# nv-tlabs/ASE

Measured on AMD Instinct MI355X. Metric: ASE PPO-update samples/sec (4096 envs x horizon 32), higher is better.
Workload: dtype f16; 1 GPU; BASELINE configs[1]: ASE agent, 4096 envs x horizon 32, obs 253 / act 31 / amp obs 1400 / latent 64, [1024,1024,512] MLPs + disc + shared-trunk encoder, minibatch 16384 (amp 4096) x 6 mini-epochs = 48 optimisation steps per update; random-init weights; precision_choice=auto without an oracle leg: the first candidate, replay=program, parallelism=single GPU

## Files before the change

ase_amd/backend.py:

```python
import ctypes as C

import torch

from . import lib as L


_HOSTFN = C.CFUNCTYPE(None, C.c_void_p)


def _ptr(t):
    return None if t is None else C.c_void_p(t.data_ptr())


def _ld(t):
    return 0 if t is None else int(t.stride(0))


def _code(dtype):
    if dtype == torch.bfloat16:
        return L.BF16
    if dtype == torch.float32:
        return L.F32
    if dtype == torch.float16:
        return L.F16
    raise L.AseHipError(f"unsupported storage dtype {dtype}")


class HipBackend:
    name = "hip"
    nt_fused_epilogue = True

    def __init__(self, device=None, x3=False):
        self.x3 = x3 if x3 == 'f16' else bool(x3)
        self._recording, self._host_keep, self._host_error = None, {}, None
        self.tn_workspace = True
        if not torch.cuda.is_available():
            raise L.AseHipError("HipBackend needs a ROCm GPU (torch.cuda.is_available() is False); "
                                "the update path has no CPU fallback")
        self.device = torch.device(device if device is not None else f"cuda:{torch.cuda.current_device()}")
        self.lib = L.get()
        self._head_scratch = torch.zeros(L.PPO_SCRATCH, dtype=torch.float64, device=self.device)
        self._head_scratch_ls = None

    def _stream(self):
        return C.c_void_p(torch.cuda.current_stream(self.device).cuda_stream)

    def zero_(self, t):
        assert t.is_contiguous()
        L.check(self.lib.ase_hip_memset(_ptr(t), 0, t.numel() * t.element_size(), self._stream()), "memset")

    def copy_(self, dst, src):
        assert dst.is_contiguous() and src.is_contiguous() and dst.dtype == src.dtype and dst.numel() == src.numel()
        L.check(self.lib.ase_hip_memcpy(_ptr(dst), _ptr(src), dst.numel() * dst.element_size(), self._stream()), "memcpy")
# ... 104 lines not shown
            row = [A.data_ptr(), _ld(A), B.data_ptr(), _ld(B), G.data_ptr(), 0 if gb is None else gb.data_ptr(), int(br),
                   M, N, K, nr, kr, ss, sd, struct.unpack('<i', struct.pack('<f', float(alpha)))[0], 0]
            for j, v in enumerate(row):
                tab[16 * i + j] = int(v)
        max_work = 8192
        work = (C.c_int32 * (4 * max_work))()
        red = (C.c_int32 * (4 * max_work))()
        n_work, n_red = C.c_int(0), C.c_int(0)
        L.check(self.lib.ase_hip_gemm_tn_grouped_plan(tab, n, int(target_wg), work, max_work, C.byref(n_work), red, max_work,
                                                      C.byref(n_red)), "gemm_tn_grouped_plan")
        nw, nr = n_work.value, n_red.value
        dev_tab = torch.tensor(list(tab), dtype=torch.int64, device=self.device)
        dev_work = torch.tensor(list(work[:4 * nw]), dtype=torch.int32, device=self.device)
        dev_red = torch.tensor(list(red[:4 * nr]), dtype=torch.int32, device=self.device)
        ws = torch.empty(nw * L.TN_SLAB, dtype=torch.float32, device=self.device) if self.tn_workspace else None
        return {'problems': dev_tab, 'work': dev_work, 'n_work': nw, 'red': dev_red, 'n_red': nr, 'ws': ws, 'keep': problems,
                'dtype': _code(problems[0][0].dtype), 'alpha_dev': alpha_dev}

    def gemm_tn_grouped(self, plan):
        L.check(self.lib.ase_hip_gemm_tn_grouped(_ptr(plan['problems']), _ptr(plan['work']), plan['n_work'], _ptr(plan['red']),
                                                 plan['n_red'], _ptr(plan['ws']), _ptr(plan.get('alpha_dev')), plan['dtype'],
                                                 self._stream()),
                "gemm_tn_grouped")

    def refresh_shadow(self, W, Ws, Wts, split_src, split_dst, x3_exp=None):
        n, k = W.shape
        ref = Ws if Ws is not None else Wts
        code = _code(ref.dtype)
        if x3_exp is not None:
            assert ref.dtype == torch.float32
            code = L.F32H3 | (int(x3_exp) << 16)
        L.check(self.lib.ase_hip_refresh_shadow(_ptr(W), n, k, _ptr(Ws), _ld(Ws), _ptr(Wts), _ld(Wts), split_src,
                                                split_dst, code, self._stream()), "refresh_shadow")

    def refresh_shadow_multi(self, desc, items, dtype):
        L.check(self.lib.ase_hip_refresh_shadow_multi(_ptr(desc), desc.shape[0], _code(dtype), self._stream()),
                "refresh_shadow_multi")

    def apply_multi(self, desc, items, dtype, opt_state, acc):
        L.check(self.lib.ase_hip_apply_multi(_ptr(desc), desc.shape[0], _ptr(opt_state), _ptr(acc), _code(dtype),
                                             self._stream()), "apply_multi")

    def apply_multi_split(self, desc, items, dtype, opt_state, acc, desc2, items2):
        assert desc2.shape == (desc.shape[0], 8) and desc2.is_contiguous()
        L.check(self.lib.ase_hip_apply_multi_v2(_ptr(desc), desc.shape[0], _ptr(desc2), _ptr(opt_state), _ptr(acc), _code(dtype),
                                                self._stream()), "apply_multi_v2")
# ... 362 lines not shown
```

ase_amd/engine.py:

```python
import contextlib
import math

import torch

from . import lib as L


def P(x, m=64):
    return (int(x) + m - 1) // m * m


_ACT = {'relu': L.ACT_RELU, 'tanh': L.ACT_TANH, 'None': L.ACT_NONE, 'none': L.ACT_NONE, None: L.ACT_NONE,
        'swish': L.ACT_SILU, 'silu': L.ACT_SILU, 'elu': L.ACT_ELU, 'gelu': L.ACT_GELU, 'sigmoid': L.ACT_SIGMOID,
        'selu': L.ACT_SELU, 'softplus': L.ACT_SOFTPLUS}
_AUX = {L.ACT_RELU: L.AUX_RELU_MASK, L.ACT_TANH: L.AUX_TANH_GRAD, L.ACT_NONE: L.AUX_NONE}
_AUX.update({a: L.AUX_PREACT | (a << 8) for a in range(L.ACT_SILU, L.ACT_SOFTPLUS + 1)})


class Dense:

    def __init__(self, parts, k_in, act, split=None):
        self.parts = parts
        self.K = k_in
        self.act = _ACT[act] if not isinstance(act, int) else act
# ... 54 lines not shown
        self.bounds_coef = float(cfg.get('bounds_loss_coef') or 0.0)
        self.adaptive_lr = cfg.get('lr_schedule', 'constant') == 'adaptive'
        self.kl_threshold = float(cfg.get('kl_threshold', 0.008))
        self.obs, self.act = net.obs_size, net.actions_num
        self.z = net.latent_dim if kind == 'ase' else 0
        self.amp = net.amp_obs_size if kind in ('amp', 'ase') else 0
        self.masked = kind in ('amp', 'ase')
        self.has_disc = kind in ('amp', 'ase')
        self.has_enc = kind == 'ase'
        self.div_on = kind == 'ase' and cfg.get('amp_diversity_bonus', 0) != 0
        self.enc_sep = bool(getattr(net, 'enc_separate', False))
        self.enc_gp = kind == 'ase' and cfg.get('enc_grad_penalty', 0) != 0 and cfg.get('enc_coef', 0) != 0
        self.mu_tanh = kind == 'ppo' and getattr(net, 'mu_tanh', False)
        self.sigma_mode = getattr(net, 'sigma_mode', 'frozen')
        self.ls_mode = {'frozen': L.LS_FROZEN, 'vector': L.LS_VECTOR, 'head': L.LS_ROWS}[self.sigma_mode]
        self.gp32 = bool(cfg.get('gp_f32', False)) and self.has_disc and dtype in (torch.float16, torch.bfloat16) and \
            cfg.get('disc_coef', 0) * cfg.get('disc_grad_penalty', 0) != 0
        self._scratch = {}
        self.multi_stream = bool(cfg.get('multi_stream', True)) and getattr(backend, 'name', '') == 'hip'
        self._side_streams = None
        o = dict(tn_grouped=True, tn_wg_side=64, tn_early=False, disc_early=True, short_prologue=True, style_early=False,
                 relu_bits=True, fused_apply=True, apply_wide=True, side_streams=2, gp_scale_split=True, xstep=True,
                 gp_stream='auto', style_side=0, style_wg=0, side_priority=None, prefetch=True, disc_after_style=False, gp_split='f16',
                 stream_offset=0, gp_value_late=False, gp_fuse='auto')
        unknown = set(cfg.get('engine_opts', {}) or {}) - set(o)
        assert not unknown, f"unknown engine_opts {sorted(unknown)}"
        o.update(cfg.get('engine_opts', {}) or {})
        self.engine_opts = o
        self._tn_defer = bool(getattr(backend, 'grouped_tn_ok', None)) and bool(o['tn_grouped'])
        self._tn_queue, self._tn_plans = [], {}
        self._tn_wg_side = int(o['tn_wg_side'])
        self._tn_early = bool(o['tn_early'])
        self._disc_early = bool(o['disc_early'])
        self._early_fork = None
        self._short_prologue = bool(o['short_prologue']) and cfg.get('graph_capture') != 'hipgraph'
        self._prep = self._lat_ready = self._fill_done = None
        self._style_early = bool(o['style_early'])
        self._n_side = max(1, min(int(o['side_streams']), 2))
        self._apply_groups = None
        self._use_bits = bool(o['relu_bits'])
        self._fused_apply = hasattr(backend, 'apply_multi') and bool(o['fused_apply'])
        self._xstep = bool(o['xstep']) and cfg.get('graph_capture') != 'hipgraph'
        gp_side = (self.dyn_scale or self.M < 8192) if o['gp_stream'] == 'auto' else bool(o['gp_stream'])
        self._gp_side = gp_side and cfg.get('graph_capture') != 'hipgraph'
        self._gp_fuse = bool(self.gp32 and getattr(backend, 'nt_fused_epilogue', False) and cfg.get('gp_f32') == 'x3'
                             and getattr(backend, 'x3', None) is not None and o['gp_split'] == 'f16'
                             and (o['gp_fuse'] == 'auto' or bool(o['gp_fuse'])))
# ... 7 lines not shown
        self._par, self._par_set, self._last_par, self._fenced = 0, False, None, False
        self._stats_exchanged = False
        self._style_wg = int(o['style_wg'])
        sp = o['side_priority']
        if sp is None:
            sp = [0, -1, 0] if (self.gp32 or self.dyn_scale) else [-1, 0, 0]
        self._side_prio = [int(x) for x in sp] if isinstance(sp, (list, tuple)) else [int(sp)] * 3
        self._gp_stream_obj = None
        self._xs = False
        self._disc_fwd_out = self._gp_value_done = self._pre_done = None
        self._apply_wide = bool(o['apply_wide'])
        self._apply_desc = self._apply_items = None
        self.force_dist = bool(cfg.get('force_dist', False))
        self.dp_grad_dtype = cfg.get('dp_grad_dtype', 'f32')
        assert self.dp_grad_dtype in ('f32', 'bf16'), self.dp_grad_dtype
        self._xbuf = {}
        self._disc_acc_mark = None
        self._merged_stats = False
        self._acc_in_bucket = False
        self._refresh_desc = None
        self._mb_desc = None
        self._mb_desc_key = None
        self._build_layers()
        self._bind_params()
        self._alloc(infer_rows)
        self.refresh_shadows()

    def _build_layers(self):
        net, z = self.net, self.z
        act = net.activation
        split = (self.obs, P(self.obs), P(self.obs) + P(z)) if z else None
        self.style = []
        if self.kind == 'ase':
            k = z
            for i, u in enumerate(net.style_units):
                self.style.append(Dense([(f'actor_mlp._style_mlp.{2 * i}', u, 0)], k, act))
                k = u
            self.style.append(Dense([('actor_mlp._style_dense', z, 0)], k, 'tanh'))
            names_a = [f'actor_mlp._dense_layers.{i}' for i in range(len(net.units))]
            names_c = [f'critic_mlp._mlp.{2 * i}' for i in range(len(net.units))]
        else:
            names_a = [f'actor_mlp.{2 * i}' for i in range(len(net.units))]
            names_c = [f'critic_mlp.{2 * i}' for i in range(len(net.units))]
        self.actor, self.critic = [], []
        k = self.obs + z
        for i, u in enumerate(net.units):
# ... 334 lines not shown
    def _mask_of(self, h):
        e = self._bits.get(h.untyped_storage().data_ptr()) if h is not None else None
        if e is None:
            return None
        base, bits = e
        off = (h.data_ptr() - base.data_ptr()) // base.element_size()
        r0, c0 = divmod(off, base.stride(0))
        if c0 != 0 or h.shape[1] != base.shape[1]:
            return None
        return bits[r0:r0 + h.shape[0]]

    def _twin(self, h, d):
        if d.act >= L.ACT_SILU:
            t = self._mask_of(h)
            assert t is not None
            return t
        return h

    def _fwd_chain(self, chain, X, H, rows):
        for d, h in zip(chain, H):
            self._fwd(d, X, h, rows)
            X = h
        return X

    def _dgrad(self, d, dY, dX, rows, aux, aux_act, wts=None, n_out=None, alpha=1.0):
        wts = d.Wts if wts is None else wts
        n_out = d.k_pad if n_out is None else n_out
        aux, mode = self._aux(aux, _AUX[aux_act])
        self._nt(dY, wts, dX, rows, n_out, d.n_pad, aux=aux, aux_mode=mode, alpha=alpha)

    def _wgrad(self, d, dY, X, rows, alpha=1.0, bias=True):
        heads = len(d.parts) > 1 or d in (self.mu_head, self.value_head, self.disc_head, self.enc_head)
        for (name, nr, off), gW, gb in zip(d.parts, d.gW, d.gb):
            self._tn(dY[:, off:], X, gW, rows, P(nr), d.k_pad, nr, d.K, d.split_src, d.split_dst, alpha=alpha,
                     gbias=gb if (bias and not heads) else None)

    def _tn(self, A, B, G, M, N, K, n_real, k_real, split_src, split_dst, alpha=1.0, gbias=None, bias_rows=0):
        br = bias_rows if bias_rows > 0 else M
        alpha = alpha / self.gs
        if self._tn_defer and self.be.grouped_tn_ok(A.dtype, M, n_real, K, br):
            self._tn_queue.append((A, B, G, gbias, br, M, N, K, n_real, k_real, split_src, split_dst, alpha))
        else:
            self.be.gemm_tn(A, B, G, M, N, K, n_real, k_real, split_src, split_dst, alpha=alpha, gbias=gbias,
                            bias_rows=bias_rows, alpha_dev=self._dI)

    def _flush_tn(self, target_wg=0):
# ... 162 lines not shown
                elif self.masked:
                    be.reduce_sum(self.mb['rand_action_mask'], M, False, self.acc, L.ACC_MASK_SUM)
                    if self._dist_shard():
                        self._ar(self.acc[L.ACC_MASK_SUM:L.ACC_MASK_SUM + 1])
            self._fill_done = None
            self._prep = prep
            self._stats_exchanged = True
            return
        be.begin_step(self.opt_state if advance else None, self.acc,
                      zero2=None if pf else (self.obs_sums if self._xs else self.stats_flat),
                      rng_bump=self.div_rng if (self.div_on and not pf) else None)
        self._prep = None
        if self._short_prologue and self._amp_stats_in_branch():
            m0 = self._mark()
            with self._Branch(self, self._side(1), m0):
                be.zero_(self.grads[:self.n_train])
                self._fill_done = self._mark()
            self._early_fork = self._fill_done if self.has_disc else None
            with self._Branch(self, self._side(0), m0) as prep:
                self.gather_minibatch(ds, idx, remap, part=2)
                if self.div_on:
                    self._draw_new_latents(new_z)
                if self.style and self._style_early:
                    sd = self.actor[0].split_dst
                    h = self._fwd_chain(self.style[:-1], self.Zs, self.Hs, self.Ra)
                    self._fwd(self.style[-1], h, self.Xa[:, sd:], self.Ra)
                self._lat_ready = self._mark()
                self.gather_minibatch(ds, idx, remap, part=1)
                if self.masked:
                    be.reduce_sum(self.mb['rand_action_mask'], M, False, self.acc, L.ACC_MASK_SUM)
            self._prep = prep
            if c.get('normalize_input', True):
                be.rms_moments(ds['obs'], self.obs, idx, remap, M, self.obs_state, self.obs_sums)
            return
        be.zero_(self.grads[:self.n_train])
        self._early_fork = self._mark() if (self.has_disc and self._amp_stats_in_branch() and self._disc_early) else None
        self.gather_minibatch(ds, idx, remap)
        if self.masked:
            be.reduce_sum(self.mb['rand_action_mask'], M, False, self.acc, L.ACC_MASK_SUM)
        if c.get('normalize_input', True):
            be.rms_moments(ds['obs'], self.obs, idx, remap, M, self.obs_state, self.obs_sums)
        if self.has_disc and not self._amp_stats_in_branch():
            self._amp_moments(amp_streams)

    def _amp_stats_in_branch(self):
        return self.multi_stream and not (self._dist_shard() and self.cfg.get('graph_capture') == 'hipgraph')

    def _dist_shard(self):
        return self._dist_on() and self.shard
# ... 166 lines not shown
            hd = he = None
        elif self._disc_fwd_out is not None:
            hd, he = self._disc_fwd_out
        elif disc_early:
            with self._Branch(self, self._side(1), fork0):
                hd, he = self._disc_forward(amp_streams)
        if self._pre_done is None:
            if norm_in:
                be.rms_finalize(self.obs_state, self.obs, self.obs_sums, self.Mg if self.shard else self.M, 1, self.obs_mean,
                                self.obs_std)
            else:
                self._identity_stats(self.obs_mean, self.obs_std)
            outs = [self.Xa[:M], self.Xc]
            if self.div_on:
                outs.append(self.Xa[M:])
            be.rms_normalize(ds['obs'], self.obs, idx, remap, M, self.obs_mean[0], self.obs_std[0], outs)
        fork1 = self._mark()
        if self._prep is not None:
            be.wait(self._lat_ready)
        elif self.div_on:
            self._draw_new_latents(new_z)

        if self.style and not (self._prep is not None and self._style_early and self._pre_done is None):
            sd = self.actor[0].split_dst
            h = self._fwd_chain(self.style[:-1], self.Zs, self.Hs, Ra)
            self._fwd(self.style[-1], h, self.Xa[:, sd:], Ra)
        style_launched = self._mark() if self._disc_fwd_out == 'split' else None
        ha = self._fwd_chain(self.actor, self.Xa, self.Ha, Ra)
        self._fwd(self.mu_head, ha, self.MU, Ra)

        with self._Branch(self, self._side(0), fork1) as br_critic:
            hc = self._fwd_chain(self.critic, self.Xc, self.Hc, M)
            self._fwd(self.value_head, hc, self.V, M)

        br_disc = None
        if self.has_disc:
            tnq, self._tn_queue = self._tn_queue, []
            with self._Branch(self, self._side(1), fork0) as br_disc:
                if self._disc_fwd_out == 'split':
                    be.wait(style_launched)
                    hd, he = self._disc_matrices()
                elif not disc_early:
                    hd, he = self._disc_forward(amp_streams)
                be.disc_head(self.HD, self.dHD, self.disc_head.gb[0], self.acc, AMB, amb_den, c['disc_coef'],
                             grad_scale=self.gs, dyn=self._dS)
                if self.has_enc:
                    src, sidx, srm = amp_streams[0]
                    zsrc = ds['ase_latents'].view(ds['ase_latents'].shape[0], -1)
                    if not self._enc_z_ready:
# ... 44 lines not shown
        self._dgrad(self.mu_head, self.dMU, self.dZa[-1], Ra, self.Ha[-1], last.act)
        self._bwd_chain(self.actor, self.Xa, self.Ha, self.dZa, Ra)
        tn_actor, self._tn_queue = self._tn_queue, []
        actor_done = self._mark()
        with self._Branch(self, self._side(0), fork2) as br_cb:
            self._wgrad(self.value_head, self.dV, hc, M)
            last = self.critic[-1]
            self._dgrad(self.value_head, self.dV, self.dZc[-1], M, self.Hc[-1], last.act)
            self._bwd_chain(self.critic, self.Xc, self.Hc, self.dZc, M)
            if self._tn_early:
                if actor_done is not None:
                    be.wait(actor_done)
                self._tn_queue = tn_actor + self._tn_queue
                self._flush_tn(0)
            else:
                tn_actor = tn_actor + self._tn_queue
                self._tn_queue = []
        def style_backward():
            a0, sdn = self.actor[0], self.style[-1]
            sd = a0.split_dst
            self._dgrad(a0, self.dZa[0], self.dStyle, Ra, self.Xa[:, sd:], sdn.act, wts=a0.Wts[sd:], n_out=P(self.z))
            hs_last = self.Hs[-1] if self.Hs else self.Zs
            self._wgrad(sdn, self.dStyle, hs_last, Ra)
            if self.Hs:
                p = self.style[-2]
                self._dgrad(sdn, self.dStyle, self.dZs[-1], Ra, self.Hs[-1], p.act)
                self._bwd_chain(self.style[:-1], self.Zs, self.Hs, self.dZs, Ra)

        if self.style and self._style_side == 2 and self.multi_stream and self._tn_defer and not self._tn_early:
            self._join_branch(br_cb)
            wide, self._tn_queue = tn_actor, []
            with self._Branch(self, self._side(0), actor_done) as br_style:
                style_backward()
            narrow, self._tn_queue = self._tn_queue, wide
            self._flush_tn(0)
            self._join_branch(br_style)
            self._tn_queue = narrow
        elif self.style and self._style_side and self.multi_stream and self._tn_defer and not self._tn_early:
            self._join_branch(br_cb)
            wide, self._tn_queue = tn_actor, []
            with self._Branch(self, self._side(0), actor_done) as br_style:
                if self._style_wg <= 0:
                    defer, self._tn_defer = self._tn_defer, False
                    style_backward()
                    self._tn_defer = defer
                else:
                    style_backward()
# ... 502 lines not shown
    def _eval_stats(self, state, D, key):
        mean, std = self._scr(key + '_m', 1, D, torch.float32), self._scr(key + '_s', 1, D, torch.float32)
        self.be.rms_finalize(state, D, None, 0, 0, mean, std)
        return mean[0], std[0]

    def _policy_nets(self, obs, z, normalize, want_mu, want_value):
        be, n = self.be, obs.shape[0]
        f32 = torch.float32
        a0 = self.actor[0]
        Xa, Xc = self._scr('Xa', n, a0.k_pad), self._scr('Xc', n, a0.k_pad)
        if normalize and self.cfg.get('normalize_input', True):
            mean, std = self._eval_stats(self.obs_state, self.obs, 'obs')
        else:
            mean, std = self._scr('one_m', 1, self.obs, f32)[0].zero_(), self._scr('one_s', 1, self.obs, f32)[0].fill_(1.0)
        be.rms_normalize(obs, self.obs, None, (0, 0), n, mean, std, [Xa, Xc])
        MU = V = None
        if self.z:
            sd = a0.split_dst
            be.gather_rows(z, self.z, None, (0, 0), n, Xc[:, sd:])
        if want_mu:
            if self.style:
                Zs = self._scr('Zs', n, P(self.z))
                be.gather_rows(z, self.z, None, (0, 0), n, Zs)
                h = Zs
                for i, d in enumerate(self.style[:-1]):
                    y = self._scr(f'Hs{i}', n, d.n_pad)
                    self._fwd(d, h, y, n)
                    h = y
                self._fwd(self.style[-1], h, Xa[:, a0.split_dst:], n)
            h = Xa
            for i, d in enumerate(self.actor):
                y = self._scr(f'Ha{i}', n, d.n_pad)
                self._fwd(d, h, y, n)
                h = y
            MU = self._scr('MU', n, self.mu_head.n_pad, f32)
            self._fwd(self.mu_head, h, MU, n)
        if want_value:
            h = Xc
            for i, d in enumerate(self.critic):
                y = self._scr(f'Hc{i}', n, d.n_pad)
                self._fwd(d, h, y, n)
                h = y
            V = self._scr('V', n, self.value_head.n_pad, f32)
            self._fwd(self.value_head, h, V, n)
        return MU, V

    def _value_out(self, V, n, unnorm_value, key='value_out'):
        v = self._scr(key, n, 1, torch.float32)
        self.be.gather_rows(V, 1, None, (0, 0), n, v)
        if unnorm_value and self.norm_value:
            self.be.rms_unnormalize(self.val_state, v, v)
        return v
# ... 140 lines not shown
```

ase_amd/lib.py:

```python
import ctypes as C
import os

_HERE = os.path.dirname(os.path.abspath(__file__))
LIB_PATH = os.path.join(_HERE, "csrc", "libase_hip.so")

ABI_VERSION = 9
PPO_SCRATCH = 1024 * 72 + 8
PPO_SCRATCH_LS = 1024 * 136 + 8
LS_FROZEN, LS_VECTOR, LS_ROWS = 0, 1, 2
TN_SLAB = 65536 + 256
F32, BF16, F32X3, F16, F32H3 = 0, 1, 2, 3, 4
ACT_NONE, ACT_RELU, ACT_TANH, ACT_SILU, ACT_ELU, ACT_GELU, ACT_SIGMOID, ACT_SELU, ACT_SOFTPLUS = range(9)
AUX_NONE, AUX_RELU_MASK, AUX_TANH_GRAD, AUX_RELU_BITS, AUX_PREACT = 0, 1, 2, 3, 4
TASK_HEADING, TASK_LOCATION, TASK_REACH, TASK_STRIKE = range(4)
TASK_OBS_COLS = (5, 2, 3, 15)
RESET_FRAME, RESET_TABLE, RESET_MOTION = range(3)
RESET_HAS_TABLE, RESET_HAS_MOTION = 1, 2

(ACC_MASK_SUM, ACC_A_LOSS, ACC_B_LOSS, ACC_ENTROPY, ACC_CLIPPED, ACC_C_LOSS, ACC_KL, ACC_DIV, ACC_BCE_AGENT,
 ACC_BCE_DEMO, ACC_AGENT_ACC, ACC_DEMO_ACC, ACC_GP, ACC_ENC, ACC_ENC_GP, ACC_LOGIT_W2, ACC_DISC_W2, ACC_ENC_W2,
 ACC_GRAD_SQ) = range(19)
ACC_COUNT = 24
(RES_A_LOSS, RES_C_LOSS, RES_B_LOSS, RES_ENTROPY, RES_CLIP_FRAC, RES_KL, RES_DISC_LOSS, RES_DISC_GP,
 RES_DISC_LOGIT_LOSS, RES_DISC_AGENT_ACC, RES_DISC_DEMO_ACC, RES_ENC_LOSS, RES_DIV_LOSS, RES_LOSS,
 RES_MASK_SUM, RES_ENC_GP, RES_LR) = range(17)
RES_COUNT = 20

_p, _i, _i64, _f, _d = C.c_void_p, C.c_int, C.c_int64, C.c_float, C.c_double

SIGNATURES = {
    "ase_hip_gemm_nt": [_p, _i64, _p, _i64, _p, _i64, _p, _p, _i64, _i, _i, _p, _i, _p, _i64, _i, _i, _i, _i, _i, _i, _f, _p, _i, _p],
    "ase_hip_gemm_nt_ex": [_p, _i64, _p, _i64, _p, _i64, _p, _p, _i64, _i, _i, _p, _i, _p, _i64, _i, _i, _i, _i, _i, _i, _f, _p, _i,
                           _p, _i, _f, _p, _i64, _i, _p, _d, _p, _p],
    "ase_hip_gemm_tn": [_p, _i64, _p, _i64, _p, _p, _i, _i, _i, _i, _i, _i, _i, _i, _f, _p, _i, _p],
    "ase_hip_refresh_shadow": [_p, _i, _i, _p, _i64, _p, _i64, _i, _i, _i, _p],
    "ase_hip_refresh_shadow_multi": [_p, _i, _i, _p],
    "ase_hip_gather_multi": [_p, _i, _p, _i, _i, _i, _p],
    "ase_hip_rms_moments": [_p, _i64, _i, _p, _i, _i, _i, _p, _p, _p],
    "ase_hip_rms_finalize": [_p, _i, _p, _p, _i, _p, _p, _p],
    "ase_hip_rms_normalize": [_p, _i64, _i, _p, _i, _i, _i, _p, _p, _p, _i64, _p, _i64, _p, _i64, _i, _p],
    "ase_hip_rms_unnormalize": [_p, _p, _p, _i64, _p],
    "ase_hip_gather_rows": [_p, _i64, _i, _p, _i, _i, _i, _p, _i64, _i, _p],
    "ase_hip_reduce_sum": [_p, _i64, _i, _p, _i, _p],
    "ase_hip_ppo_head": [_p, _i64, _p, _i64] + [_p] * 11 + [_p, _i64, _p, _i64, _p, _p, _p, _p, _p] + [_i] * 8 + [_f] * 6 + [_p]
                        + [_i, _i64, _p, _i64, _p, _f] + [_i, _p],
    "ase_hip_disc_head": [_p, _i64, _p, _i64, _p, _p, _i, _i, _f, _f, _p, _i, _p],
    "ase_hip_enc_head": [_p, _i64, _p, _i64, _p, _i64, _p, _p, _p, _i, _i, _i, _f, _f, _p, _i, _p],
    "ase_hip_gp_seed": [_p, _i64, _p, _p, _i64, _i, _i, _f, _i, _i, _p],
    "ase_hip_gp_second": [_p, _i64, _p, _i64, _p, _i64, _p, _i64, _i, _i, _i, _i, _p],
    "ase_hip_colsum": [_p, _i64, _i, _i, _f, _p, _p],
    "ase_hip_sqnorm": [_p, _i64, _i, _i, _p, _i, _d, _p, _i, _p],
    "ase_hip_finalize_scalars": [_p, _p, _i, _i, _i, _i, _i, _i] + [_f] * 11 + [_p, _f, _p],
    "ase_hip_enc_gp_seed": [_p, _i64, _p, _i64, _p, _i64, _i, _i, _f, _i, _p],
    "ase_hip_enc_gp_back": [_p, _i64, _p, _i64, _p, _i64, _p, _i64, _p, _i, _i, _f, _p, _i, _p],
    "ase_hip_clip_scale": [_p, _i64, _p, _f, _p],
    "ase_hip_begin_step": [_p, _p, _i, _p, _i, _p, _p],
# ... 83 lines not shown
```

include/ase_hip.h:

```cpp
#ifndef ASE_HIP_H
#define ASE_HIP_H

#include <stdint.h>

#ifdef __cplusplus
extern "C" {
#endif

#define ASE_HIP_ABI_VERSION 9

enum { ASE_F32 = 0, ASE_BF16 = 1, ASE_F32X3 = 2 ,
       ASE_F32H3 = 4 ,
       ASE_F16 = 3  };
enum { ASE_ACT_NONE = 0, ASE_ACT_RELU = 1, ASE_ACT_TANH = 2, ASE_ACT_SILU = 3, ASE_ACT_ELU = 4, ASE_ACT_GELU = 5,
       ASE_ACT_SIGMOID = 6, ASE_ACT_SELU = 7, ASE_ACT_SOFTPLUS = 8 };
enum { ASE_AUX_NONE = 0, ASE_AUX_RELU_MASK = 1, ASE_AUX_TANH_GRAD = 2, ASE_AUX_RELU_BITS = 3 ,
       ASE_AUX_PREACT = 4  };
enum { ASE_OK = 0, ASE_EINVAL = -1, ASE_ELAUNCH = -2, ASE_EUNSUPPORTED = -3 };

int ase_hip_abi_version(void);
const char* ase_hip_last_error(void);

int ase_hip_gemm_nt_kernel_id(int M, int N, int K, int dtype);

int ase_hip_debug_nt_profile(void* buf);
int ase_hip_debug_nt_profile_clock(int shader_clock);


int ase_hip_gemm_nt(const void* A, int64_t lda, const void* B, int64_t ldb, void* C, int64_t ldc,
                    const float* bias, const void* aux, int64_t ldaux, int aux_split, int aux_delta,
                    float* colsum, int colsum_n, void* mask_out, int64_t ldmask, int M, int N, int K, int act,
                    int aux_mode, int out_f32, float alpha, float* alpha_dev, int dtype, void* stream);

int ase_hip_gemm_nt_ex(const void* A, int64_t lda, const void* B, int64_t ldb, void* C, int64_t ldc,
                       const float* bias, const void* aux, int64_t ldaux, int aux_split, int aux_delta,
                       float* colsum, int colsum_n, void* mask_out, int64_t ldmask, int M, int N, int K, int act,
                       int aux_mode, int out_f32, float alpha, float* alpha_dev, int dtype,
                       const float* seed_w, int seed_n, float seed_scale, void* twin, int64_t ldtwin, int twin_dtype,
                       double* sq_acc, double sq_scale, const float* sq_dyn, void* stream);

int ase_hip_gemm_tn(const void* A, int64_t lda, const void* B, int64_t ldb, float* G, float* gbias,
                    int bias_rows, int M, int N, int K, int n_real, int k_real, int split_src, int split_dst,
                    float alpha, const float* alpha_dev, int dtype, void* stream);

#define ASE_TN_SLAB (65536 + 256)
int ase_hip_gemm_tn_grouped_plan(int64_t* problems, int n_problems, int target_wg, int32_t* work, int max_work,
                                 int* n_work, int32_t* red, int max_red, int* n_red);
int ase_hip_gemm_tn_grouped(const int64_t* problems, const int32_t* work, int n_work, const int32_t* red, int n_red,
                            float* workspace, const float* alpha_dev, int dtype, void* stream);

int ase_hip_refresh_shadow(const float* W, int n_real, int k_real, void* Ws, int64_t ldws,
                           void* Wts, int64_t ldwts, int split_src, int split_dst, int dtype,
                           void* stream);

int ase_hip_refresh_shadow_multi(const int64_t* desc, int n_layers, int dtype, void* stream);


int ase_hip_rms_moments(const float* src, int64_t ld_src, int D, const int32_t* idx, int remap_h,
                        int remap_n, int M, const double* state, double* sums, void* stream);

int ase_hip_rms_moments_multi(const float* const* srcs, const int64_t* ld_srcs, const int32_t* const* idxs,
                              const int* remap_h, const int* remap_n, double* const* sums, int n_streams, int D, int M,
// ... 225 lines not shown
```

Before: 1.825 million samples/s.

## Fuse three-layer style MLP forward and backward dgrad into single HIP kernels

```diff
diff --git a/ase_amd/backend.py b/ase_amd/backend.py
--- a/ase_amd/backend.py
+++ b/ase_amd/backend.py
@@ -29,6 +29,7 @@
 class HipBackend:
     name = "hip"
     nt_fused_epilogue = True
+    style_mlp_fused = True
 
     def __init__(self, device=None, x3=False):
         self.x3 = x3 if x3 == 'f16' else bool(x3)
@@ -179,6 +180,30 @@
                                                  plan['n_red'], _ptr(plan['ws']), _ptr(plan.get('alpha_dev')), plan['dtype'],
                                                  self._stream()),
                 "gemm_tn_grouped")
+
+    def style_mlp_ok(self, dtype, k0, n1, n2, act1, act2, act3):
+        if dtype not in (torch.float16, torch.bfloat16):
+            return False
+        return bool(self.lib.ase_hip_style_mlp_ok(_code(dtype), int(k0), int(n1), int(n2), int(act1), int(act2), int(act3)))
+
+    def style_mlp_fwd(self, Z, W1, b1, W2, b2, W3, b3, Y, rows, k0, H1=None, M1=None, H2=None, M2=None,
+                      acts=(L.ACT_RELU, L.ACT_RELU, L.ACT_TANH)):
+        assert W1.dtype == Z.dtype and W2.dtype == Z.dtype and W3.dtype == Z.dtype and Y.dtype == Z.dtype
+        assert all(m is None or m.dtype == torch.int32 for m in (M1, M2))
+        assert all(h is None or h.dtype == Z.dtype for h in (H1, H2))
+        L.check(self.lib.ase_hip_style_mlp_fwd(_ptr(Z), _ld(Z), _ptr(W1), _ld(W1), _ptr(b1), _ptr(W2), _ld(W2), _ptr(b2), _ptr(W3),
+                                               _ld(W3), _ptr(b3), _ptr(H1), _ld(H1), _ptr(M1), _ld(M1), _ptr(H2), _ld(H2), _ptr(M2),
+                                               _ld(M2), _ptr(Y), _ld(Y), int(rows), int(k0), W1.shape[0], W2.shape[0],
+                                               int(acts[0]), int(acts[1]), int(acts[2]), _code(Z.dtype), self._stream()),
+                "style_mlp_fwd")
+
+    def style_mlp_bwd(self, dY, Wt3, Wt2, M2, M1, dZ2, dZ1, rows, k0, acts=(L.ACT_RELU, L.ACT_RELU)):
+        assert Wt3.dtype == dY.dtype and Wt2.dtype == dY.dtype and dZ2.dtype == dY.dtype and dZ1.dtype == dY.dtype
+        assert M1.dtype == torch.int32 and M2.dtype == torch.int32
+        L.check(self.lib.ase_hip_style_mlp_bwd(_ptr(dY), _ld(dY), _ptr(Wt3), _ld(Wt3), _ptr(Wt2), _ld(Wt2), _ptr(M2), _ld(M2), _ptr(M1),
+                                               _ld(M1), _ptr(dZ2), _ld(dZ2), _ptr(dZ1), _ld(dZ1), int(rows), int(k0), Wt2.shape[0],
+                                               Wt3.shape[0], int(acts[0]), int(acts[1]), _code(dY.dtype), self._stream()),
+                "style_mlp_bwd")
 
     def refresh_shadow(self, W, Ws, Wts, split_src, split_dst, x3_exp=None):
         n, k = W.shape
diff --git a/ase_amd/csrc/style_mlp.hip b/ase_amd/csrc/style_mlp.hip
--- /dev/null
+++ b/ase_amd/csrc/style_mlp.hip
@@ -0,0 +1,418 @@
+#include "gemm_nt_kernels.h"
+
+namespace {
+
+using namespace ase_nt;
+
+constexpr int SM_ROWS = 128, SM_N1 = 512, SM_N2 = 256;
+
+struct StyleFwdParams {
+    const char* Z; int64_t ldz;
+    const char* W1; int64_t ldw1;
+    const char* W2; int64_t ldw2;
+    const char* W3; int64_t ldw3;
+    const float *b1, *b2, *b3;
+    char* H1; int64_t ldh1;
+    uint32_t* M1; int64_t ldm1;
+    char* H2; int64_t ldh2;
+    uint32_t* M2; int64_t ldm2;
+    char* Y; int64_t ldy;
+    int rows;
+};
+
+struct StyleBwdParams {
+    const char* dY; int64_t lddy;
+    const char* Wt3; int64_t ldwt3;
+    const char* Wt2; int64_t ldwt2;
+    const uint32_t* M2; int64_t ldm2;
+    const uint32_t* M1; int64_t ldm1;
+    char* dZ2; int64_t lddz2;
+    char* dZ1; int64_t lddz1;
+    int rows;
+};
+
+template <int RB, int ROWS>
+__device__ __forceinline__ void sm_stage(const char* src, int64_t ld, int row0, int row_max, int koff, char* dst, int wid, int lane) {
+    constexpr int RPP = 1024 / RB, CPR = RB / 16;
+#pragma unroll
+    for (int q0 = 0; q0 < ROWS / RPP; q0 += 8) {
+        const int q = q0 + wid;
+        if (q < ROWS / RPP) {
+            const int r = q * RPP + lane / CPR, slot = lane % CPR;
+            const char* g = src + (int64_t)min(row0 + r, row_max) * ld + koff + ((slot ^ lds_swz<RB>(r)) << 4);
+            __builtin_amdgcn_global_load_lds((gptr_t*)g, (lptr_t*)(dst + q * 1024), 16, 0, 0);
+        }
+    }
+}
+
+__device__ __forceinline__ void sm_sync_dma() {
+    asm volatile("s_waitcnt vmcnt(0) lgkmcnt(0)" ::: "memory");
+    NT8_BARRIER();
+}
+__device__ __forceinline__ void sm_sync_lds() {
+    asm volatile("s_waitcnt lgkmcnt(0)" ::: "memory");
+    NT8_BARRIER();
+}
+
+__device__ __forceinline__ void sm_runs(const uint32_t (&pk)[4][2], uint4 (&out)[2]) {
+#pragma unroll
+    for (int g = 0; g < 4; g += 2) {
+        const auto s0 = __builtin_amdgcn_permlane32_swap(pk[g][0], pk[g + 1][0], false, false);
+        const auto s1 = __builtin_amdgcn_permlane32_swap(pk[g][1], pk[g + 1][1], false, false);
+        out[g >> 1] = make_uint4(s0[0], s1[0], s0[1], s1[1]);
+    }
+}
+__device__ __forceinline__ void sm_put(const uint4 (&out)[2], char* grow, bool ok, char* lrow, int jj, int sw, int h) {
+#pragma unroll
+    for (int t = 0; t < 2; ++t) {
+        if (lrow) {
+            const uint32_t a = (uint32_t)(uintptr_t)lrow + (uint32_t)(((jj * 4 + 2 * t + h) ^ sw) << 4);
+            const i32x4 d = {(int)out[t].x, (int)out[t].y, (int)out[t].z, (int)out[t].w};
+            asm volatile("ds_write_b128 %0, %1" : : "v"(a), "v"(d) : "memory");
+        }
+        if (ok) *reinterpret_cast<uint4*>(grow + (16 * t + 8 * h) * 2) = out[t];
+    }
+}
+__device__ __forceinline__ uint32_t sm_mask_word(uint32_t mb) {
+    const auto w = __builtin_amdgcn_permlane32_swap(mb, mb, false, false);
+    return w[0] | w[1];
+}
+
+template <typename T, int RB> __device__ __forceinline__ typename V16<T>::x8 sm_frag(const char* image, int row, int kchunk) {
+    return *reinterpret_cast<const typename V16<T>::x8*>(image + row * RB + ((kchunk ^ lds_swz<RB>(row)) << 4));
+}
+
+__device__ __forceinline__ void sm_zero(f32x16& a) {
+#pragma unroll
+    for (int e = 0; e < 16; ++e) a[e] = 0.f;
+}
+
+constexpr int FW_W2 = 0;
+constexpr int FW_H1 = 65536;
+constexpr int FW_W1 = 81920;
+constexpr int FW_Z = 98304;
+constexpr int FW_W3 = 114688;
+constexpr int FW_B = 147456;
+constexpr int FW_LDS = FW_B + (SM_N1 + SM_N2 + 64) * 4;
+
+template <typename T, int K0>
+__global__ __launch_bounds__(512) void style_mlp_fwd_kernel(StyleFwdParams p) {
+    typedef typename V16<T>::x8 x8;
+    constexpr int RB0 = K0 * 2, KS0 = K0 / 16, NJ3 = K0 / 32;
+    extern __shared__ __attribute__((aligned(16))) char smem[];
+    const int tid = threadIdx.x, lane = tid & 63;
+    const int wid = __builtin_amdgcn_readfirstlane(tid >> 6);
+    const int r = lane & 31, h = lane >> 5, sw = lds_swz<128>(r);
+    const int row0 = blockIdx.x * SM_ROWS, rmax = p.rows - 1;
+    float* sB = reinterpret_cast<float*>(smem + FW_B);
+
+    for (int i = tid; i < SM_N1 + SM_N2 + K0; i += 512)
+        sB[i] = i < SM_N1 ? p.b1[i] : (i < SM_N1 + SM_N2 ? p.b2[i - SM_N1] : p.b3[i - SM_N1 - SM_N2]);
+    asm volatile("s_waitcnt vmcnt(0)" ::: "memory");
+    sm_stage<RB0, SM_ROWS>(p.Z, p.ldz, row0, rmax, 0, smem + FW_Z, wid, lane);
+#pragma unroll
+    for (int kt = 0; kt < 4; ++kt) sm_stage<128, K0>(p.W3, p.ldw3, 0, K0 - 1, kt * 128, smem + FW_W3 + kt * K0 * 128, wid, lane);
+    sm_stage<RB0, 64>(p.W1, p.ldw1, 0, SM_N1 - 1, 0, smem + FW_W1, wid, lane);
+    sm_stage<128, SM_N2>(p.W2, p.ldw2, 0, SM_N2 - 1, 0, smem + FW_W2, wid, lane);
+    sm_sync_dma();
+
+    const int i1 = wid >> 1, j1 = wid & 1;
+    const int wr = wid >> 2, wc = wid & 3;
+    x8 zf[KS0];
+#pragma unroll
+    for (int ks = 0; ks < KS0; ++ks) zf[ks] = sm_frag<T, RB0>(smem + FW_Z, i1 * 32 + r, ks * 2 + h);
+
+    f32x16 acc2[2][2];
+#pragma unroll
+    for (int i = 0; i < 2; ++i)
+#pragma unroll
+        for (int j = 0; j < 2; ++j) sm_zero(acc2[i][j]);
+    const f32x2 one = {1.f, 1.f};
+    const i16x2 relu_lo = {0, 0};
+    const int m1 = row0 + i1 * 32 + r;
+    const bool ok1 = m1 < p.rows;
+
+    for (int c = 0; c < SM_N1 / 64; ++c) {
+        if (c > 0) sm_sync_dma();
+        const char* w1 = smem + FW_W1 + (c & 1) * 8192;
+        const char* w2 = smem + FW_W2 + (c & 1) * 32768;
+        x8 bf[KS0];
+#pragma unroll
+        for (int ks = 0; ks < KS0; ++ks) bf[ks] = sm_frag<T, RB0>(w1, j1 * 32 + r, ks * 2 + h);
+        f32x4 bias[4];
+#pragma unroll
+        for (int g = 0; g < 4; ++g) bias[g] = *reinterpret_cast<const f32x4*>(sB + c * 64 + j1 * 32 + 8 * g + 4 * h);
+        asm volatile("s_waitcnt lgkmcnt(0)" ::: "memory");
+        __builtin_amdgcn_sched_barrier(0);
+        if (c + 1 < SM_N1 / 64) {
+            sm_stage<RB0, 64>(p.W1, p.ldw1, (c + 1) * 64, SM_N1 - 1, 0, smem + FW_W1 + ((c + 1) & 1) * 8192, wid, lane);
+            sm_stage<128, SM_N2>(p.W2, p.ldw2, 0, SM_N2 - 1, (c + 1) * 128, smem + FW_W2 + ((c + 1) & 1) * 32768, wid, lane);
+        }
+        __builtin_amdgcn_sched_barrier(0);
+        f32x16 a1;
+        sm_zero(a1);
+#pragma unroll
+        for (int ks = 0; ks < KS0; ++ks) a1 = mfma16<T>(bf[ks], zf[ks], a1);
+        uint32_t pk[4][2];
+        const uint32_t mb = rows_frag<T, 0, true>(a1, bias, 0u, one, relu_lo, h, pk);
+        uint4 out[2];
+        sm_runs(pk, out);
+        const int n0 = c * 64 + j1 * 32;
+        sm_put(out, p.H1 + (int64_t)m1 * p.ldh1 + n0 * 2, ok1 && p.H1 != nullptr, smem + FW_H1 + (i1 * 32 + r) * 128, j1, sw, h);
+        const uint32_t word = sm_mask_word(mb);
+        if (p.M1 && ok1 && h == 0) p.M1[(int64_t)m1 * p.ldm1 + (n0 >> 5)] = word;
+        sm_sync_lds();
+        Mma<T>::template tile<2, 2, 128, true>(smem + FW_H1 + wr * 64 * 128, w2 + wc * 64 * 128, lane, acc2);
+    }
+    sm_sync_lds();
+
+#pragma unroll
+    for (int j = 0; j < 2; ++j) {
+        f32x4 bias[4];
+#pragma unroll
+        for (int g = 0; g < 4; ++g) bias[g] = *reinterpret_cast<const f32x4*>(sB + SM_N1 + wc * 64 + j * 32 + 8 * g + 4 * h);
+#pragma unroll
+        for (int i = 0; i < 2; ++i) {
+            const int lr = wr * 64 + i * 32 + r, m = row0 + lr, n0 = wc * 64 + j * 32;
+            const bool ok = m < p.rows;
+            uint32_t pk[4][2];
+            const uint32_t mb = rows_frag<T, 0, true>(acc2[i][j], bias, 0u, one, relu_lo, h, pk);
+            uint4 out[2];
+            sm_runs(pk, out);
+            sm_put(out, p.H2 + (int64_t)m * p.ldh2 + n0 * 2, ok && p.H2 != nullptr, smem + FW_W2 + wc * 16384 + lr * 128, j, sw, h);
+            const uint32_t word = sm_mask_word(mb);
+            if (p.M2 && ok && h == 0) p.M2[(int64_t)m * p.ldm2 + (n0 >> 5)] = word;
+        }
+    }
+    sm_sync_lds();
+
+    const int i3 = wid / NJ3, j3 = wid % NJ3;
+    if (i3 < 4) {
+        f32x16 a3;
+        sm_zero(a3);
+#pragma unroll
+        for (int kt = 0; kt < 4; ++kt)
+#pragma unroll
+            for (int ks = 0; ks < 4; ++ks) {
+                const x8 a = sm_frag<T, 128>(smem + FW_W2 + kt * 16384, i3 * 32 + r, ks * 2 + h);
+                const x8 b = sm_frag<T, 128>(smem + FW_W3 + kt * K0 * 128, j3 * 32 + r, ks * 2 + h);
+                a3 = mfma16<T>(b, a, a3);
+            }
+        uint32_t pk[4][2];
+#pragma unroll
+        for (int g = 0; g < 4; ++g) {
+            const f32x4 b = *reinterpret_cast<const f32x4*>(sB + SM_N1 + SM_N2 + j3 * 32 + 8 * g + 4 * h);
+#pragma unroll
+            for (int pr = 0; pr < 2; ++pr) {
+                const T lo = from_f32<T>(tanhf(1.f * a3[g * 4 + 2 * pr] + b[2 * pr]));
+                const T hi = from_f32<T>(tanhf(1.f * a3[g * 4 + 2 * pr + 1] + b[2 * pr + 1]));
+                pk[g][pr] = (uint32_t)__builtin_bit_cast(unsigned short, lo) | ((uint32_t)__builtin_bit_cast(unsigned short, hi) << 16);
+            }
+        }
+        uint4 out[2];
+        sm_runs(pk, out);
+        const int m = row0 + i3 * 32 + r;
+        sm_put(out, p.Y + (int64_t)m * p.ldy + j3 * 32 * 2, m < p.rows, nullptr, 0, 0, h);
+    }
+}
+
+constexpr int BW_W = 0;
+constexpr int BW_DZ2 = 65536;
+constexpr int BW_DY = 131072;
+constexpr int BW_LDS = 147456;
+
+template <typename T, int K0>
+__global__ __launch_bounds__(512) void style_mlp_bwd_kernel(StyleBwdParams p) {
+    typedef typename V16<T>::x8 x8;
+    constexpr int RB0 = K0 * 2, NCH = SM_N1 / 64;
+    extern __shared__ __attribute__((aligned(16))) char smem[];
+    const int tid = threadIdx.x, lane = tid & 63;
+    const int wid = __builtin_amdgcn_readfirstlane(tid >> 6);
+    const int r = lane & 31, h = lane >> 5, sw = lds_swz<128>(r);
+    const int row0 = blockIdx.x * SM_ROWS, rmax = p.rows - 1;
+    const int wr = wid >> 2, wc = wid & 3;
+    const int i2 = wid >> 1, j2 = wid & 1;
+
+    uint32_t bits2[2][2], bits1[NCH];
+#pragma unroll
+    for (int i = 0; i < 2; ++i)
+#pragma unroll
+        for (int j = 0; j < 2; ++j)
+            bits2[i][j] = p.M2[(int64_t)min(row0 + wr * 64 + i * 32 + r, rmax) * p.ldm2 + wc * 2 + j];
+#pragma unroll
+    for (int c = 0; c < NCH; ++c) bits1[c] = p.M1[(int64_t)min(row0 + i2 * 32 + r, rmax) * p.ldm1 + c * 2 + j2];
+    asm volatile("s_waitcnt vmcnt(0)" : "+v"(bits2[0][0]), "+v"(bits2[0][1]), "+v"(bits2[1][0]), "+v"(bits2[1][1]) : : "memory");
+    asm volatile("" : "+v"(bits1[0]), "+v"(bits1[1]), "+v"(bits1[2]), "+v"(bits1[3]), "+v"(bits1[4]), "+v"(bits1[5]), "+v"(bits1[6]),
+                 "+v"(bits1[7]) : : "memory");
+
+    sm_stage<RB0, SM_ROWS>(p.dY, p.lddy, row0, rmax, 0, smem + BW_DY, wid, lane);
+    sm_stage<RB0, SM_N2>(p.Wt3, p.ldwt3, 0, SM_N2 - 1, 0, smem + BW_W + 32768, wid, lane);
+#pragma unroll
+    for (int kt = 0; kt < 4; ++kt) sm_stage<128, 64>(p.Wt2, p.ldwt2, 0, SM_N1 - 1, kt * 128, smem + BW_W + kt * 8192, wid, lane);
+    sm_sync_dma();
+
+    const f32x2 one = {1.f, 1.f};
+    const i16x2 none_lo = {(short)-32768, (short)-32768};
+    f32x4 zero4[4];
+#pragma unroll
+    for (int g = 0; g < 4; ++g) zero4[g] = f32x4{0.f, 0.f, 0.f, 0.f};
+    {
+        f32x16 acc[2][2];
+#pragma unroll
+        for (int i = 0; i < 2; ++i)
+#pragma unroll
+            for (int j = 0; j < 2; ++j) sm_zero(acc[i][j]);
+        Mma<T>::template tile<2, 2, RB0, true>(smem + BW_DY + wr * 64 * RB0, smem + BW_W + 32768 + wc * 64 * RB0, lane, acc);
+#pragma unroll
+        for (int i = 0; i < 2; ++i)
+#pragma unroll
+            for (int j = 0; j < 2; ++j) {
+                const int lr = wr * 64 + i * 32 + r, m = row0 + lr, n0 = wc * 64 + j * 32;
+                uint32_t pk[4][2];
+                rows_frag<T, 2, false>(acc[i][j], zero4, bits2[i][j] >> (4 * h), one, none_lo, h, pk);
+                uint4 out[2];
+                sm_runs(pk, out);
+                sm_put(out, p.dZ2 + (int64_t)m * p.lddz2 + n0 * 2, m < p.rows, smem + BW_DZ2 + wc * 16384 + lr * 128, j, sw, h);
+            }
+    }
+    sm_sync_lds();
+
+    x8 af[16];
+#pragma unroll
+    for (int kt = 0; kt < 4; ++kt)
+#pragma unroll
+        for (int ks = 0; ks < 4; ++ks) af[kt * 4 + ks] = sm_frag<T, 128>(smem + BW_DZ2 + kt * 16384, i2 * 32 + r, ks * 2 + h);
+    const int m2 = row0 + i2 * 32 + r;
+    const bool ok2 = m2 < p.rows;
+
+    for (int c = 0; c < NCH; ++c) {
+        if (c > 0) sm_sync_dma();
+        const char* w = smem + BW_W + (c & 1) * 32768;
+        x8 bf[16];
+#pragma unroll
+        for (int kt = 0; kt < 4; ++kt)
+#pragma unroll
+            for (int ks = 0; ks < 4; ++ks) bf[kt * 4 + ks] = sm_frag<T, 128>(w + kt * 8192, j2 * 32 + r, ks * 2 + h);
+        asm volatile("s_waitcnt lgkmcnt(0)" ::: "memory");
+        __builtin_amdgcn_sched_barrier(0);
+        if (c + 1 < NCH) {
+#pragma unroll
+            for (int kt = 0; kt < 4; ++kt)
+                sm_stage<128, 64>(p.Wt2, p.ldwt2, (c + 1) * 64, SM_N1 - 1, kt * 128, smem + BW_W + ((c + 1) & 1) * 32768 + kt * 8192, wid, lane);
+        }
+        __builtin_amdgcn_sched_barrier(0);
+        f32x16 a;
+        sm_zero(a);
+#pragma unroll
+        for (int k = 0; k < 16; ++k) a = mfma16<T>(bf[k], af[k], a);
+        uint32_t pk[4][2];
+        rows_frag<T, 2, false>(a, zero4, bits1[c] >> (4 * h), one, none_lo, h, pk);
+        uint4 out[2];
+        sm_runs(pk, out);
+        sm_put(out, p.dZ1 + (int64_t)m2 * p.lddz1 + (c * 64 + j2 * 32) * 2, ok2, nullptr, 0, 0, h);
+    }
+}
+
+bool style_shape_ok(int dtype, int k0, int n1, int n2, int act1, int act2, int act3) {
+    return (dtype == ASE_F16 || dtype == ASE_BF16) && (k0 == 32 || k0 == 64) && n1 == SM_N1 && n2 == SM_N2 && act1 == ASE_ACT_RELU &&
+           act2 == ASE_ACT_RELU && act3 == ASE_ACT_TANH;
+}
+
+template <typename K> int style_set_lds(K kern, int lds, const char* name) {
+    hipError_t e = hipFuncSetAttribute(reinterpret_cast<const void*>(kern), hipFuncAttributeMaxDynamicSharedMemorySize, lds);
+    if (e != hipSuccess) {
+        ase_set_error("%s: hipFuncSetAttribute failed: %s", name, hipGetErrorString(e));
+        return ASE_ELAUNCH;
+    }
+    return ASE_OK;
+}
+
+template <typename T, int K0> int launch_style_fwd(const StyleFwdParams& p, hipStream_t stream) {
+    static bool attr_done = false;
+    auto kern = style_mlp_fwd_kernel<T, K0>;
+    if (!attr_done) {
+        if (int rc = style_set_lds(kern, FW_LDS, "style_mlp_fwd")) return rc;
+        attr_done = true;
+    }
+    ASE_LAUNCH(kern, dim3((p.rows + SM_ROWS - 1) / SM_ROWS), dim3(512), FW_LDS, stream, p);
+    ASE_CHECK_LAUNCH("style_mlp_fwd");
+    return ASE_OK;
+}
+
+template <typename T, int K0> int launch_style_bwd(const StyleBwdParams& p, hipStream_t stream) {
+    static bool attr_done = false;
+    auto kern = style_mlp_bwd_kernel<T, K0>;
+    if (!attr_done) {
+        if (int rc = style_set_lds(kern, BW_LDS, "style_mlp_bwd")) return rc;
+        attr_done = true;
+    }
+    ASE_LAUNCH(kern, dim3((p.rows + SM_ROWS - 1) / SM_ROWS), dim3(512), BW_LDS, stream, p);
+    ASE_CHECK_LAUNCH("style_mlp_bwd");
+    return ASE_OK;
+}
+
+inline bool al16(const void* q, int64_t ld_elems) { return ((uintptr_t)q % 16) == 0 && (ld_elems * 2) % 16 == 0; }
+
+}
+
+extern "C" int ase_hip_style_mlp_ok(int dtype, int k0, int n1, int n2, int act1, int act2, int act3) {
+    return style_shape_ok(dtype, k0, n1, n2, act1, act2, act3) ? 1 : 0;
+}
+
+extern "C" int ase_hip_style_mlp_fwd(const void* Z, int64_t ldz, const void* W1, int64_t ldw1, const float* b1, const void* W2,
+                                     int64_t ldw2, const float* b2, const void* W3, int64_t ldw3, const float* b3, void* H1,
+                                     int64_t ldh1, void* M1, int64_t ldm1, void* H2, int64_t ldh2, void* M2, int64_t ldm2, void* Y,
+                                     int64_t ldy, int rows, int k0, int n1, int n2, int act1, int act2, int act3, int dtype,
+                                     void* stream) {
+    ASE_CHECK_ARG(style_shape_ok(dtype, k0, n1, n2, act1, act2, act3),
+                  "style_mlp_fwd: f16 / bf16 storage, k0 32 or 64, widths 512 / 256, ReLU, ReLU, tanh only (dtype=%d k0=%d n1=%d n2=%d "
+                  "act=%d,%d,%d)", dtype, k0, n1, n2, act1, act2, act3);
+    ASE_CHECK_ARG(Z && W1 && b1 && W2 && b2 && W3 && b3 && Y && rows > 0, "style_mlp_fwd: null/empty operand (rows=%d)", rows);
+    ASE_CHECK_ARG(ldz >= k0 && ldw1 >= k0 && ldw2 >= n1 && ldw3 >= n2 && ldy >= k0 && (!H1 || ldh1 >= n1) && (!H2 || ldh2 >= n2),
+                  "style_mlp_fwd: leading dimension too small");
+    ASE_CHECK_ARG(al16(Z, ldz) && al16(W1, ldw1) && al16(W2, ldw2) && al16(W3, ldw3) && al16(Y, ldy) && (!H1 || al16(H1, ldh1)) &&
+                      (!H2 || al16(H2, ldh2)) && ((uintptr_t)b1 % 4) == 0 && ((uintptr_t)b2 % 4) == 0 && ((uintptr_t)b3 % 4) == 0,
+                  "style_mlp_fwd: matrices must be 16-byte aligned with 16-byte row pitch");
+    ASE_CHECK_ARG((!M1 || (H1 && ((uintptr_t)M1 % 4) == 0 && ldm1 * 32 >= n1)) && (!M2 || (H2 && ((uintptr_t)M2 % 4) == 0 && ldm2 * 32 >= n2)),
+                  "style_mlp_fwd: a mask matrix needs its activation buffer and ldm >= n / 32 words");
+    ASE_CHECK_ARG((int64_t)rows * ldz < (int64_t)0x3FFFFFFF, "style_mlp_fwd: too many rows");
+    StyleFwdParams p;
+    p.Z = (const char*)Z; p.ldz = ldz * 2;
+    p.W1 = (const char*)W1; p.ldw1 = ldw1 * 2;
+    p.W2 = (const char*)W2; p.ldw2 = ldw2 * 2;
+    p.W3 = (const char*)W3; p.ldw3 = ldw3 * 2;
+    p.b1 = b1; p.b2 = b2; p.b3 = b3;
+    p.H1 = (char*)H1; p.ldh1 = ldh1 * 2; p.M1 = (uint32_t*)M1; p.ldm1 = ldm1;
+    p.H2 = (char*)H2; p.ldh2 = ldh2 * 2; p.M2 = (uint32_t*)M2; p.ldm2 = ldm2;
+    p.Y = (char*)Y; p.ldy = ldy * 2;
+    p.rows = rows;
+    hipStream_t s = (hipStream_t)stream;
+    if (dtype == ASE_F16) return k0 == 64 ? launch_style_fwd<f16_t, 64>(p, s) : launch_style_fwd<f16_t, 32>(p, s);
+    return k0 == 64 ? launch_style_fwd<bf16_t, 64>(p, s) : launch_style_fwd<bf16_t, 32>(p, s);
+}
+
+extern "C" int ase_hip_style_mlp_bwd(const void* dY, int64_t lddy, const void* Wt3, int64_t ldwt3, const void* Wt2, int64_t ldwt2,
+                                     const void* M2, int64_t ldm2, const void* M1, int64_t ldm1, void* dZ2, int64_t lddz2, void* dZ1,
+                                     int64_t lddz1, int rows, int k0, int n1, int n2, int act1, int act2, int dtype, void* stream) {
+    ASE_CHECK_ARG(style_shape_ok(dtype, k0, n1, n2, act1, act2, ASE_ACT_TANH),
+                  "style_mlp_bwd: f16 / bf16 storage, k0 32 or 64, widths 512 / 256, ReLU, ReLU only (dtype=%d k0=%d n1=%d n2=%d act=%d,%d)",
+                  dtype, k0, n1, n2, act1, act2);
+    ASE_CHECK_ARG(dY && Wt3 && Wt2 && M2 && M1 && dZ2 && dZ1 && rows > 0, "style_mlp_bwd: null/empty operand (rows=%d)", rows);
+    ASE_CHECK_ARG(lddy >= k0 && ldwt3 >= k0 && ldwt2 >= n2 && lddz2 >= n2 && lddz1 >= n1 && ldm2 * 32 >= n2 && ldm1 * 32 >= n1,
+                  "style_mlp_bwd: leading dimension too small");
+    ASE_CHECK_ARG(al16(dY, lddy) && al16(Wt3, ldwt3) && al16(Wt2, ldwt2) && al16(dZ2, lddz2) && al16(dZ1, lddz1) &&
+                      ((uintptr_t)M1 % 4) == 0 && ((uintptr_t)M2 % 4) == 0,
+                  "style_mlp_bwd: matrices must be 16-byte aligned with 16-byte row pitch");
+    StyleBwdParams p;
+    p.dY = (const char*)dY; p.lddy = lddy * 2;
+    p.Wt3 = (const char*)Wt3; p.ldwt3 = ldwt3 * 2;
+    p.Wt2 = (const char*)Wt2; p.ldwt2 = ldwt2 * 2;
+    p.M2 = (const uint32_t*)M2; p.ldm2 = ldm2;
+    p.M1 = (const uint32_t*)M1; p.ldm1 = ldm1;
+    p.dZ2 = (char*)dZ2; p.lddz2 = lddz2 * 2;
+    p.dZ1 = (char*)dZ1; p.lddz1 = lddz1 * 2;
+    p.rows = rows;
+    hipStream_t s = (hipStream_t)stream;
+    if (dtype == ASE_F16) return k0 == 64 ? launch_style_bwd<f16_t, 64>(p, s) : launch_style_bwd<f16_t, 32>(p, s);
+    return k0 == 64 ? launch_style_bwd<bf16_t, 64>(p, s) : launch_style_bwd<bf16_t, 32>(p, s);
+}
diff --git a/ase_amd/engine.py b/ase_amd/engine.py
--- a/ase_amd/engine.py
+++ b/ase_amd/engine.py
@@ -100,7 +100,7 @@
         o = dict(tn_grouped=True, tn_wg_side=64, tn_early=False, disc_early=True, short_prologue=True, style_early=False,
                  relu_bits=True, fused_apply=True, apply_wide=True, side_streams=2, gp_scale_split=True, xstep=True,
                  gp_stream='auto', style_side=0, style_wg=0, side_priority=None, prefetch=True, disc_after_style=False, gp_split='f16',
-                 stream_offset=0, gp_value_late=False, gp_fuse='auto')
+                 stream_offset=0, gp_value_late=False, gp_fuse='auto', style_fuse='auto')
         unknown = set(cfg.get('engine_opts', {}) or {}) - set(o)
         assert not unknown, f"unknown engine_opts {sorted(unknown)}"
         o.update(cfg.get('engine_opts', {}) or {})
@@ -154,6 +154,11 @@
         self._mb_desc = None
         self._mb_desc_key = None
         self._build_layers()
+        sf, st = o['style_fuse'], self.style
+        assert sf == 'auto' or sf is True or sf is False, f"engine_opts style_fuse: 'auto', True or False, not {sf!r}"
+        self._style_fuse = bool(sf is not False and len(st) == 3 and not self.dyn_scale and self._use_bits
+                                and getattr(backend, 'style_mlp_fused', False) and st[2].n_pad == st[0].k_pad
+                                and backend.style_mlp_ok(dtype, st[0].k_pad, st[0].n_pad, st[1].n_pad, st[0].act, st[1].act, st[2].act))
         self._bind_params()
         self._alloc(infer_rows)
         self.refresh_shadows()
@@ -534,6 +539,23 @@
             self._fwd(d, X, h, rows)
             X = h
         return X
+
+    def _style_forward(self, Z, Hs, Y, rows):
+        st = self.style
+        if self._style_fuse and len(st) == 3:
+            h1, h2 = Hs if Hs is not None else (None, None)
+            self.be.style_mlp_fwd(Z, st[0].Ws, st[0].bs, st[1].Ws, st[1].bs, st[2].Ws, st[2].bs, Y, rows, st[0].k_pad,
+                                  H1=h1, M1=self._mask_of(h1), H2=h2, M2=self._mask_of(h2), acts=(st[0].act, st[1].act, st[2].act))
+            return
+        if Hs is None:
+            Hs = [self._scr(f'Hs{i}', rows, d.n_pad) for i, d in enumerate(st[:-1])]
+        h = self._fwd_chain(st[:-1], Z, Hs, rows)
+        self._fwd(st[-1], h, Y, rows)
+
+    def _style_dgrad(self, rows):
+        st = self.style
+        self.be.style_mlp_bwd(self.dStyle, st[2].Wts, st[1].Wts, self._mask_of(self.Hs[1]), self._mask_of(self.Hs[0]),
+                              self.dZs[1], self.dZs[0], rows, st[0].k_pad, acts=(st[0].act, st[1].act))
 
     def _dgrad(self, d, dY, dX, rows, aux, aux_act, wts=None, n_out=None, alpha=1.0):
         wts = d.Wts if wts is None else wts
@@ -742,9 +764,7 @@
                 if self.div_on:
                     self._draw_new_latents(new_z)
                 if self.style and self._style_early:
-                    sd = self.actor[0].split_dst
-                    h = self._fwd_chain(self.style[:-1], self.Zs, self.Hs, self.Ra)
-                    self._fwd(self.style[-1], h, self.Xa[:, sd:], self.Ra)
+                    self._style_forward(self.Zs, self.Hs, self.Xa[:, self.actor[0].split_dst:], self.Ra)
                 self._lat_ready = self._mark()
                 self.gather_minibatch(ds, idx, remap, part=1)
                 if self.masked:
@@ -957,9 +977,7 @@
             self._draw_new_latents(new_z)
 
         if self.style and not (self._prep is not None and self._style_early and self._pre_done is None):
-            sd = self.actor[0].split_dst
-            h = self._fwd_chain(self.style[:-1], self.Zs, self.Hs, Ra)
-            self._fwd(self.style[-1], h, self.Xa[:, sd:], Ra)
+            self._style_forward(self.Zs, self.Hs, self.Xa[:, self.actor[0].split_dst:], Ra)
         style_launched = self._mark() if self._disc_fwd_out == 'split' else None
         ha = self._fwd_chain(self.actor, self.Xa, self.Ha, Ra)
         self._fwd(self.mu_head, ha, self.MU, Ra)
@@ -1050,7 +1068,11 @@
             self._dgrad(a0, self.dZa[0], self.dStyle, Ra, self.Xa[:, sd:], sdn.act, wts=a0.Wts[sd:], n_out=P(self.z))
             hs_last = self.Hs[-1] if self.Hs else self.Zs
             self._wgrad(sdn, self.dStyle, hs_last, Ra)
-            if self.Hs:
+            if self._style_fuse:
+                self._style_dgrad(Ra)
+                self._wgrad(self.style[1], self.dZs[1], self.Hs[0], Ra)
+                self._wgrad(self.style[0], self.dZs[0], self.Zs, Ra)
+            elif self.Hs:
                 p = self.style[-2]
                 self._dgrad(sdn, self.dStyle, self.dZs[-1], Ra, self.Hs[-1], p.act)
                 self._bwd_chain(self.style[:-1], self.Zs, self.Hs, self.dZs, Ra)
@@ -1599,12 +1621,7 @@
             if self.style:
                 Zs = self._scr('Zs', n, P(self.z))
                 be.gather_rows(z, self.z, None, (0, 0), n, Zs)
-                h = Zs
-                for i, d in enumerate(self.style[:-1]):
-                    y = self._scr(f'Hs{i}', n, d.n_pad)
-                    self._fwd(d, h, y, n)
-                    h = y
-                self._fwd(self.style[-1], h, Xa[:, a0.split_dst:], n)
+                self._style_forward(Zs, None, Xa[:, a0.split_dst:], n)
             h = Xa
             for i, d in enumerate(self.actor):
                 y = self._scr(f'Ha{i}', n, d.n_pad)
diff --git a/ase_amd/lib.py b/ase_amd/lib.py
--- a/ase_amd/lib.py
+++ b/ase_amd/lib.py
@@ -32,6 +32,10 @@
     "ase_hip_gemm_nt": [_p, _i64, _p, _i64, _p, _i64, _p, _p, _i64, _i, _i, _p, _i, _p, _i64, _i, _i, _i, _i, _i, _i, _f, _p, _i, _p],
     "ase_hip_gemm_nt_ex": [_p, _i64, _p, _i64, _p, _i64, _p, _p, _i64, _i, _i, _p, _i, _p, _i64, _i, _i, _i, _i, _i, _i, _f, _p, _i,
                            _p, _i, _f, _p, _i64, _i, _p, _d, _p, _p],
+    "ase_hip_style_mlp_ok": [_i] * 7,
+    "ase_hip_style_mlp_fwd": [_p, _i64, _p, _i64, _p, _p, _i64, _p, _p, _i64, _p, _p, _i64, _p, _i64, _p, _i64, _p, _i64, _p, _i64]
+                             + [_i] * 8 + [_p],
+    "ase_hip_style_mlp_bwd": [_p, _i64, _p, _i64, _p, _i64, _p, _i64, _p, _i64, _p, _i64, _p, _i64] + [_i] * 7 + [_p],
     "ase_hip_gemm_tn": [_p, _i64, _p, _i64, _p, _p, _i, _i, _i, _i, _i, _i, _i, _i, _f, _p, _i, _p],
     "ase_hip_refresh_shadow": [_p, _i, _i, _p, _i64, _p, _i64, _i, _i, _i, _p],
     "ase_hip_refresh_shadow_multi": [_p, _i, _i, _p],
diff --git a/include/ase_hip.h b/include/ase_hip.h
--- a/include/ase_hip.h
+++ b/include/ase_hip.h
@@ -38,6 +38,15 @@
                        int aux_mode, int out_f32, float alpha, float* alpha_dev, int dtype,
                        const float* seed_w, int seed_n, float seed_scale, void* twin, int64_t ldtwin, int twin_dtype,
                        double* sq_acc, double sq_scale, const float* sq_dyn, void* stream);
+
+int ase_hip_style_mlp_ok(int dtype, int k0, int n1, int n2, int act1, int act2, int act3);
+int ase_hip_style_mlp_fwd(const void* Z, int64_t ldz, const void* W1, int64_t ldw1, const float* b1, const void* W2, int64_t ldw2,
+                          const float* b2, const void* W3, int64_t ldw3, const float* b3, void* H1, int64_t ldh1, void* M1,
+                          int64_t ldm1, void* H2, int64_t ldh2, void* M2, int64_t ldm2, void* Y, int64_t ldy, int rows, int k0,
+                          int n1, int n2, int act1, int act2, int act3, int dtype, void* stream);
+int ase_hip_style_mlp_bwd(const void* dY, int64_t lddy, const void* Wt3, int64_t ldwt3, const void* Wt2, int64_t ldwt2,
+                          const void* M2, int64_t ldm2, const void* M1, int64_t ldm1, void* dZ2, int64_t lddz2, void* dZ1,
+                          int64_t lddz1, int rows, int k0, int n1, int n2, int act1, int act2, int dtype, void* stream);
 
 int ase_hip_gemm_tn(const void* A, int64_t lda, const void* B, int64_t ldb, float* G, float* gbias,
                     int bias_rows, int M, int N, int K, int n_real, int k_real, int split_src, int split_dst,
```

Result: slower. 1.787 million samples/s (-2.1%).
